# LoganWilliams1/mhm2_kmer_analysis_v2

Measured on AMD Instinct MI355X. Metric: k-mers/sec (kcount stage) at k=21, higher is better.
Workload: dtype u64

## Files before the change

### mhm2_kmer_analysis_v2_amd/csrc/kc_bucketed.hpp

```cpp
#pragma once
#include "kc_kernels.hpp"

namespace kc {

constexpr int WGB = 1024;
constexpr int SUPER_SPAN = 16 * WGB - PRE - POST;
using TileSuper = TileGeo<WGB, SUPER_SPAN>;
static_assert(TileSuper::GPT == 1 && TileSuper::NGROUP == WGB, "one group per thread");
constexpr int PMAX = 1024;
constexpr int GMAX = 512;

template <int NL> struct Rnd {
  static constexpr int RPOS = NL == 1 ? 16 : NL == 2 ? 8 : 4;
  static constexpr int RPOS_READS = NL == 1 ? 8 : NL <= 3 ? 4 : 2;
  static constexpr size_t STAGE = ((size_t)WGB * RPOS + 64) * NL * 8;
  static constexpr size_t STAGE_READS = ((size_t)WGB * RPOS_READS + 64) * NL * 8;
};

struct Geom {
  uint32_t G, P1, P2, S;
  uint32_t log2CH1, log2CH2;
  uint32_t L1MAX, L2MAX;
  uint32_t A1;
  uint32_t A2;
// ... 1327 lines not shown
  const uint32_t CH1m = (1u << gm.log2CH1) - 1u;
  const uint8_t *const rec1 = reinterpret_cast<const uint8_t *>(bb.rec1);
  for (uint32_t b1 = (FL ? fs.b_lo : 0u) + blockIdx.x; b1 < (FL ? fs.b_hi : P1); b1 += gridDim.x) {
    {
      const int tid = fresh_tid();
      uint32_t v = 0;
      if ((uint32_t)tid < G) {
        const uint32_t cnt = bb.cnt1[(size_t)tid * P1 + b1];
        uint32_t d = 0;
        if constexpr (INC) {
          d = bb.done1[(size_t)tid * P1 + b1];
          L.skip[tid] = d;
        }
        L.end[tid] = cnt;
        v = cnt > d ? ((cnt - (d & ~1u) + 1u) & ~1u) : 0u;
      }
      if constexpr (FL) {
        if ((uint32_t)tid >= G && (uint32_t)tid < GT) {
          const uint32_t c = fs.cnt[(size_t)(tid - G) * fs.nbo + (b1 - fs.b_lo)];
          L.flo[tid - G] = fs.at[(size_t)(tid - G) * fs.nbo + (b1 - fs.b_lo)];
          L.end[tid] = c;
          v = (c + 1u) & ~1u;
        }
      }
      const uint32_t e = block_excl_scan(v, L.sp.scan);
      if ((uint32_t)tid < GT) L.pre[tid] = e;
      if (tid == 0) L.pre[GT] = L.sp.scan.total;
    }
    ChainDest D;
    D.arena = bb.rec2;
    D.chain = bb.chain2 + (size_t)b1 * P2 * gm.L2MAX;
    D.log2CH = gm.log2CH2;
    D.LMAX = gm.L2MAX;
    D.arena_base = (uint32_t)__builtin_amdgcn_readfirstlane((int)bb.base2[b1]);
    D.arena_cap = (uint32_t)__builtin_amdgcn_readfirstlane((int)(bb.base2[b1 + 1] - bb.base2[b1]));
    D.own_lo = 0;
    D.own_hi = PMAX;
#ifdef KC_STAMPS
    unsigned long long tprev_ = __builtin_amdgcn_s_memtime();
    D.stamps = cb + 8;
    D.tprev = &tprev_;
#endif
    ChainState cst = split_load_state(L.sp, P2, INC ? bb.cnt2 + (size_t)b1 * P2 : nullptr, D.chain, D.LMAX, D.log2CH, INC ? bb.used2[b1] : 0u);
    __syncthreads();
    const uint32_t n = L.pre[GT];
    const uint32_t half = WGB * RPOS;
    uint32_t p_ids = 0, p_rec = 0;
    uint32_t nxa[NPAIR], nxb[NPAIR], nxc[NPAIR];
    uint32_t nxt_valid = 0, nxt_flat = 0;
    auto load_half = [&](uint32_t v0) __attribute__((always_inline)) {
      const uint32_t t = (uint32_t)fresh_tid();
      uint32_t ids[NPAIR];
#pragma unroll
      for (int j = 0; j < NPAIR; j++) {
        const uint32_t e = min(v0 + 2u * ((uint32_t)j * WGB + t), n - 2u);
        while (e >= L.pre[p_ids + 1]) p_ids++;
        const uint32_t i0 = e - L.pre[p_ids] + (INC ? (L.skip[p_ids] & ~1u) : 0u);
        const size_t ci = ((size_t)p_ids * gm.P1 + b1) * gm.L1MAX + (i0 >> gm.log2CH1);
        ids[j] = bb.chain1[FL && p_ids >= G ? 0 : ci];
      }
      nxt_valid = 0;
#pragma unroll
      for (int j = 0; j < NPAIR; j++) {
        const uint32_t ev = v0 + 2u * ((uint32_t)j * WGB + t), e = min(ev, n - 2u);
        while (e >= L.pre[p_rec + 1]) p_rec++;
        const bool flat = FL && p_rec >= G;
        const uint32_t first = (INC && !flat) ? L.skip[p_rec] : 0u;
        const uint32_t i0 = e - L.pre[p_rec] + (first & ~1u), end = L.end[p_rec];
        const uint8_t *src = rec1 + ((((size_t)p_rec * gm.A1 + ids[j]) << gm.log2CH1) + (i0 & CH1m)) * 6;
        if constexpr (FL) {
          const uint64_t f0 = L.flo[flat ? p_rec - G : 0u];
          if (flat) src = reinterpret_cast<const uint8_t *>((uintptr_t)f0) + 5u * (size_t)i0;
          nxt_flat = flat ? (nxt_flat | (1u << j)) : (nxt_flat & ~(1u << j));
        }
        const bool in = ev < n;
        nxt_valid |= (in && i0 >= first && i0 < end ? 1u : 0u) << (2 * j);
        nxt_valid |= (in && i0 + 1u < end ? 2u : 0u) << (2 * j);
        const Load12 w = *reinterpret_cast<const Load12 *>(src);
        nxa[j] = w.a;
        nxb[j] = w.b;
        nxc[j] = w.c;
      }
    };
    auto request = [&](uint64_t v0) __attribute__((always_inline)) {
      if (v0 < n) load_half((uint32_t)v0);
      else nxt_valid = 0;
    };
    uint32_t lo[RPOS], br[RPOS];
    uint32_t cur_valid = 0;
    const uint32_t sh_b2 = gm.k2 - gm.la - gm.lb;
    auto take_over = [&]() __attribute__((always_inline)) {
#pragma unroll
      for (int j = 0; j < NPAIR; j++) {
        const Load12 w = {nxa[j], nxb[j], nxc[j]};
        uint32_t e0, e1;
        if (FL && ((nxt_flat >> j) & 1u)) {
          lo[2 * j] = w.a;
          e0 = w.b & 63u;
          lo[2 * j + 1] = (w.b >> 8) | (w.c << 24);
          e1 = (w.c >> 8) & 63u;
        } else {
          lo[2 * j] = w.a;
          e0 = (w.b >> 10) & 63u;
          lo[2 * j + 1] = (w.b >> 16) | (w.c << 16);
          e1 = w.c >> 26;
        }
        br[2 * j] = ((lo[2 * j] >> sh_b2) & (P2 - 1u)) | (e0 << 10);
        br[2 * j + 1] = ((lo[2 * j + 1] >> sh_b2) & (P2 - 1u)) | (e1 << 10);
      }
      cur_valid = nxt_valid;
    };
    auto rank_half = [&](int buf) __attribute__((always_inline)) {
#pragma unroll
      for (int j = 0; j < RPOS; j++) {
        const bool valid = (cur_valid >> j) & 1u;
        const uint32_t rank = hist_rank(L.sp, buf, br[j] & (PMAX - 1), valid);
        br[j] = valid ? (br[j] | (rank << 16)) : ~0u;
      }
    };
    const uint32_t rb_mask = (1u << sh_b2) - 1u;
    auto scatter_half = [&](const uint32_t *at) __attribute__((always_inline)) {
#pragma unroll
      for (int j0 = 0; j0 < RPOS; j0 += 8) {
        uint32_t pos[8];
#pragma unroll
        for (int j = 0; j < 8; j++) pos[j] = at[br[j0 + j] & (PMAX - 1)];
#pragma unroll
        for (int j = 0; j < 8; j++) {
          const uint32_t bj = br[j0 + j];
          const uint32_t p = bj != ~0u ? pos[j] + (bj >> 16) : L2R6_ROUND + lane_id();
          staged[p] = ((lo[j0 + j] & rb_mask) << 6) | ((bj >> 10) & 63u);
        }
      }
    };
    uint32_t *const arena32 = reinterpret_cast<uint32_t *>(D.arena);
    const size_t arena0 = (size_t)D.arena_base << D.log2CH;
    if (n) load_half(0);
    take_over();
    request(half);
    int buf = 0;
    bool second = false;
    uint32_t a1 = 0, total1 = 0;
    for (uint32_t v0 = 0; v0 < n || second; v0 += half) {
      rank_half(buf);
      KC_SPLIT_STAMP(0)
      lds_barrier();
      uint32_t S = 0, o_hi = 0;
      {
        const int tid = fresh_tid();
        KC_SPLIT_STAMP(1)
        const uint32_t c = (uint32_t)tid < P2 ? L.sp.hist[buf][tid] : 0u;
        const uint32_t e = block_excl_scan(c, L.sp.scan);
        if (!second) {
          if ((uint32_t)tid < P2) L.sp.hist[buf ^ 1][tid] = e;
          a1 = c | (e << 16);
        } else {
          S = e;
          o_hi = (uint32_t)__builtin_amdgcn_readlane((int)(e + c), 63);
          if ((uint32_t)tid < P2) {
            const RunPlace q = split_reserve(L.sp, (uint32_t)tid, c, S, D, cst);
            L.sp.dst[tid] = make_uint4(q.x, q.y, q.fit | (q.w << 16), a1);
            L.sp.hist[buf][tid] = total1 + S - (a1 >> 16) - (a1 & 0xFFFFu);
            L.sp.hist[buf ^ 1][tid] = 0;
          }
        }
        lds_barrier();
        if (!second) total1 = (uint32_t)__builtin_amdgcn_readfirstlane((int)L.sp.scan.total);
        KC_SPLIT_STAMP(2)
      }
      scatter_half(second ? L.sp.hist[buf] : L.sp.hist[buf ^ 1]);
      if (second) lds_barrier();
      KC_SPLIT_STAMP(3)
      take_over();
      request(v0 + 2 * (uint64_t)half);
      KC_SPLIT_STAMP(5)
      if (second) {
        const int tid = fresh_tid();
        const uint32_t wave = (uint32_t)__builtin_amdgcn_readfirstlane(tid >> 6), lane = lane_id();
        uint32_t r0 = wave * 64u, Sl = S;
        if (P2 < (uint32_t)WGB) {
          if ((uint32_t)tid < P2) L.sp.hist[buf][tid] = S;
          lds_barrier();
          const uint32_t G = (P2 + 15u) >> 4, total = L.sp.scan.total;
          r0 = min(wave * G, P2);
          const uint32_t r1 = min(r0 + G, P2), r = min(r0 + lane, r1);
          Sl = r < r1 ? L.sp.hist[buf][r] : ~0u;
          o_hi = (uint32_t)__builtin_amdgcn_readfirstlane((int)(r1 < P2 ? L.sp.hist[buf][r1] : total));
        }
        const uint32_t o_lo = (uint32_t)__builtin_amdgcn_readlane((int)Sl, 0);
        constexpr int U = 4;
        for (uint32_t o0 = o_lo; o0 < o_hi; o0 += U * 64) {
          uint32_t oc[U], r[U], s[U], word[U];
          uint4 d[U];
#pragma unroll
          for (int u = 0; u < U; u++) {
            const uint32_t ou = min(o0 + 64u * u, o_hi - 1u);
            oc[u] = min(ou + lane, o_hi - 1u);
            const uint64_t le = __ballot(Sl <= ou);
            uint32_t l = 63u - (uint32_t)__clzll((long long)le);
            r[u] = l;
            s[u] = (uint32_t)__builtin_amdgcn_readlane((int)Sl, (int)l);
            for (uint64_t m = __ballot(Sl > ou && Sl - ou < 64u); m; m &= m - 1u) {
              l = (uint32_t)__builtin_ctzll(m);
              const uint32_t sl = (uint32_t)__builtin_amdgcn_readlane((int)Sl, (int)l);
              if (oc[u] >= sl) {
                r[u] = l;
                s[u] = sl;
              }
            }
          }
#pragma unroll
          for (int u = 0; u < U; u++) d[u] = L.sp.dst[r0 + r[u]];
#pragma unroll
          for (int u = 0; u < U; u++) {
            const uint32_t j = oc[u] - s[u], n1 = d[u].w & 0xFFFFu, st1 = d[u].w >> 16;
            word[u] = staged[j < n1 ? st1 + j : total1 + oc[u] - st1 - n1];
          }
          bool spill = false;
#pragma unroll
          for (int u = 0; u < U; u++) {
            const uint32_t j = oc[u] - s[u];
            const bool live = o0 + 64u * u + lane < o_hi, fits = j < (d[u].z & 0xFFFFu);
            const uint32_t at = (j < (d[u].z >> 16) ? d[u].x : d[u].y) + oc[u];
            if (live && fits) arena32[arena0 + at] = word[u];
            spill |= live && !fits;
          }
          if (__any(spill)) {
#pragma unroll
            for (int u = 0; u < U; u++) {
              if (o0 + 64u * u + lane < o_hi && oc[u] - s[u] >= (d[u].z & 0xFFFFu)) {
                const size_t reg = (size_t)b1 * P2 + r0 + r[u];
                bb.flag[reg] = 1;
                const uint64_t o = atomicAdd((unsigned long long *)&cb[CB_OVF2], 1ULL);
                if (o < bb.ovf2_cap) bb.ovf2[o] = cp_unpack_rec(word[u], reg, gm);
                else atomicOr((unsigned long long *)&cb[CB_FATAL], (unsigned long long)FATAL_OVF2);
              }
            }
          }
        }
        KC_SPLIT_STAMP(4)
        buf ^= 1;
      }
      second = !second;
    }
    {
      const int tid = fresh_tid();
      if ((uint32_t)tid < P2) bb.cnt2[(size_t)b1 * P2 + tid] = cst.cur;
      if constexpr (INC) {
        if ((uint32_t)tid < G) bb.done1[(size_t)tid * P1 + b1] = L.end[tid];
        if (tid == 0) bb.used2[b1] = min(L.sp.arena_used, D.arena_cap);
      }
    }
    __syncthreads();
  }
}

template <int NL, bool CP>
__global__ void kc_ovf1_to_regions_kernel(Geom gm, BucketBufs bb, uint64_t n, uint64_t *cb) {
  const uint64_t i = (uint64_t)blockIdx.x * blockDim.x + threadIdx.x;
  if (i >= n) return;
  uint64_t r[NL];
  for (int w = 0; w < NL; w++) r[w] = bb.ovf1[i * NL + w];
  size_t reg;
  if (CP) {
    const uint64_t m = cp_mix_rec(r[0], gm);
    reg = (size_t)cp_b1(m, gm) * gm.P2 + cp_b2(m, gm);
  } else {
    const uint64_t h = rec_hash<NL>(r);
    reg = (size_t)hash_b1(h, gm) * gm.P2 + hash_b2(h, gm);
  }
  bb.flag[reg] = 1;
  const uint64_t o = atomicAdd((unsigned long long *)&cb[CB_OVF2], 1ULL);
  if (o < bb.ovf2_cap) {
    for (int w = 0; w < NL; w++) bb.ovf2[o * NL + w] = r[w];
  } else {
    atomicOr((unsigned long long *)&cb[CB_FATAL], (unsigned long long)FATAL_OVF2);
  }
}

template <int NL, bool CP>
__global__ __launch_bounds__(TPB) void kc_ovf1_drain_kernel(Geom gm, BucketBufs bb, uint64_t n, Table t, uint64_t *ctrs) {
  for (uint64_t i = (uint64_t)blockIdx.x * TPB + threadIdx.x; i < n; i += (uint64_t)gridDim.x * TPB) {
    uint64_t r[NL];
    for (int w = 0; w < NL; w++) r[w] = bb.ovf1[i * NL + w];
    size_t reg;
    if (CP) {
      const uint64_t m = cp_mix_rec(r[0], gm);
      reg = (size_t)cp_b1(m, gm) * gm.P2 + cp_b2(m, gm);
    } else {
      const uint64_t h = rec_hash<NL>(r);
      reg = (size_t)hash_b1(h, gm) * gm.P2 + hash_b2(h, gm);
    }
    bb.flag[reg] = 1;
    table_insert<NL>(t, r, ctrs);
  }
}

constexpr uint32_t CHAIN_LDS = 480;

template <int NL>
struct CountLDS {
  static constexpr uint32_t SMAX = NL <= 2 ? 4096 : 2048;
  static constexpr int ew(bool) { return NL == 1 ? 6 : 5; }
  uint32_t chain[2][CHAIN_LDS];
  uint32_t hdr[2][2];
  uint32_t nout;
  uint32_t ncand;
  uint32_t fail[2];
  uint32_t gbase_lo, gbase_hi, gbase2_lo, gbase2_hi, split;
  static constexpr size_t header_bytes() { return (sizeof(CountLDS<NL>) + 15) & ~size_t(15); }
  static constexpr size_t bytes(uint32_t S, bool cp) { return header_bytes() + (size_t)S * ((cp ? 4 : 8 * NL) + 4 * ew(cp) + 2) + 16; }
};
static_assert(2 * CountLDS<2>::bytes(2048, false) <= 160 * 1024, "two workgroups of the two-word count kernel per CU");

struct CountTab {
  uint64_t *keys;
  uint32_t *ext;
  uint16_t *cand;
  uint32_t S, lgS;
};

template <int NL, bool CP>
__device__ __forceinline__ CountTab count_tab(uint8_t *smem, uint32_t S) {
  CountTab t;
  uint8_t *p = smem + CountLDS<NL>::header_bytes();
  t.keys = reinterpret_cast<uint64_t *>(p);
  p += (size_t)S * (CP ? 4 : 8 * NL);
  t.ext = reinterpret_cast<uint32_t *>(p);
  p += (size_t)S * 4 * CountLDS<NL>::ew(CP);
  t.cand = reinterpret_cast<uint16_t *>(p);
  t.S = S;
  t.lgS = 31u - (uint32_t)__clz(S);
  return t;
}

template <int EW>
__device__ __forceinline__ void ext_count(const CountTab &tb, uint32_t s, uint32_t le, uint32_t re) {
  if constexpr (EW == 6) {
    le = min(le, 4u);
    re = min(re, 4u);
    atomicAdd(&tb.ext[((le >> 1) << tb.lgS) + s], 1u << ((le & 1u) << 4));
    atomicAdd(&tb.ext[((3u + (re >> 1)) << tb.lgS) + s], 1u << ((re & 1u) << 4));
  } else {
    const bool nl = (le & 4u) != 0, nr = (re & 4u) != 0;
    const uint32_t wl = nl ? 4u : (le >> 1), wr = nr ? 4u : 2u + (re >> 1);
    const uint32_t il = nl ? 1u : 1u << ((le & 1u) << 4), ir = nr ? 0x10000u : 1u << ((re & 1u) << 4);
    atomicAdd(&tb.ext[(wl << tb.lgS) + s], il);
    atomicAdd(&tb.ext[(wr << tb.lgS) + s], ir);
  }
}
template <int EW>
__device__ __forceinline__ uint32_t ext_get(const uint32_t *ext, uint32_t SM, uint32_t s, uint32_t side, uint32_t e) {
  return (ext[((EW == 6 ? 3 : 2) * side + (e >> 1)) * SM + s] >> (16 * (e & 1u))) & 0xFFFFu;
}

struct OutBufs {
  uint64_t *keys;
  uint16_t *counts;
  uint8_t *left, *right;
  uint16_t *exts;
  uint64_t cap;
  uint64_t *cursor;
  uint32_t block;
  uint64_t *tails;
};

__device__ __forceinline__ uint32_t lds_probe1(unsigned long long *claim, uint32_t Sm1, uint64_t key, uint32_t slot, uint32_t valid,
                                               uint32_t &failed) {
  uint32_t act = valid;
  const uint32_t klo = (uint32_t)key, khi = (uint32_t)(key >> 32);
  uint32_t trips = 0;
  do {
    unsigned long long old = key;
    if (act) old = atomicCAS(&claim[slot], (unsigned long long)KEY_EMPTY, (unsigned long long)key);
    const uint32_t olo = (uint32_t)old, ohi = (uint32_t)(old >> 32);
    const uint32_t differs = (olo ^ klo) | (ohi ^ khi);
    const uint32_t notempty = ~(olo & ohi);
    const uint32_t miss = min(differs, notempty) ? act : 0u;
    act = miss;
    slot = (slot + miss) & Sm1;
    if (++trips > Sm1 + 1) {
      failed |= act;
      break;
    }
  } while (__any(act));
  return slot;
}

__device__ __forceinline__ uint32_t lds_probe32(uint32_t *claim, uint32_t Sm1, uint32_t key, uint32_t slot, uint32_t stride, bool valid,
                                                uint32_t &failed) {
#ifndef KC_PROBE_CXX
  uint32_t at = slot << 2, old, addr, trips = Sm1 + 2;
  const uint32_t m4 = Sm1 << 2, step = stride << 2;
  const uint32_t base = (uint32_t)(uintptr_t)claim;
  const uint64_t live = __builtin_amdgcn_ballot_w64(valid);
  uint64_t sv, t;
  asm volatile(
      "s_mov_b64 %[sv], exec\n\t"
      "s_and_b64 exec, exec, %[live]\n\t"
      "s_cbranch_execz 2f\n"
      "1:\n\t"
      "v_add_u32_e32 %[addr], %[base], %[at]\n\t"
      "ds_cmpst_rtn_b32 %[old], %[addr], %[empty], %[key]\n\t"
      "s_waitcnt lgkmcnt(0)\n\t"
      "v_cmp_ne_u32_e32 vcc, %[old], %[key]\n\t"
      "v_cmp_ne_u32_e64 %[t], -1, %[old]\n\t"
      "s_and_b64 vcc, vcc, %[t]\n\t"
      "s_and_b64 exec, exec, vcc\n\t"
      "s_cbranch_execz 2f\n\t"
      "v_add_u32_e32 %[at], %[step], %[at]\n\t"
      "v_and_b32_e32 %[at], %[m4], %[at]\n\t"
      "s_sub_u32 %[trips], %[trips], 1\n\t"
      "s_cmp_lg_u32 %[trips], 0\n\t"
      "s_cbranch_scc1 1b\n\t"
      "v_mov_b32_e32 %[fl], 1\n"
      "2:\n\t"
      "s_mov_b64 exec, %[sv]\n\t"
      : [old] "=&v"(old), [addr] "=&v"(addr), [at] "+v"(at), [fl] "+v"(failed), [trips] "+s"(trips), [sv] "=&s"(sv), [t] "=&s"(t)
      : [live] "s"(live), [base] "s"(base), [empty] "v"(0xFFFFFFFFu), [key] "v"(key), [step] "v"(step), [m4] "s"(m4)
      : "vcc", "scc", "memory");
  return at >> 2;
#else
  uint32_t trips = 0, at = slot << 2;
  const uint32_t m4 = Sm1 << 2, step = stride << 2;
  bool go = valid;
  do {
    uint32_t old = key;
    if (go) old = atomicCAS(reinterpret_cast<uint32_t *>(reinterpret_cast<char *>(claim) + at), 0xFFFFFFFFu, key);
    go = go & (old != key) & (old != 0xFFFFFFFFu);
    at = (at + (go ? step : 0u)) & m4;
    if (++trips > Sm1 + 1) {
      failed |= go ? 1u : 0u;
      break;
    }
  } while (__builtin_amdgcn_ballot_w64(go) != 0);
  return at >> 2;
#endif
}

template <int NL>
__device__ __forceinline__ uint32_t lds_probeN(const CountTab &tb, const uint64_t (&key)[NL], uint32_t slot, uint32_t valid, uint32_t &failed);

__device__ __forceinline__ uint32_t lds_probe2(const CountTab &tb, uint64_t key0, uint64_t klast, uint32_t slot, bool valid, uint32_t &failed) {
#ifndef KC_PROBE2_CXX
  const uint32_t m8 = (tb.S - 1u) << 3;
  uint32_t at = slot << 3, a0, a1, trips = 4u * tb.S + 2u;
  const uint32_t base0 = (uint32_t)(uintptr_t)tb.keys, base1 = base0 + (tb.S << 3);
  const uint64_t live = __builtin_amdgcn_ballot_w64(valid);
  const uint64_t empty = KEY_EMPTY, busy = KEY_BUSY;
  uint64_t old, w0, sv, act, won, t1, t2;
  asm volatile(
      "s_mov_b64 %[sv], exec\n\t"
      "s_and_b64 %[act], exec, %[live]\n\t"
      "s_mov_b64 exec, %[act]\n\t"
      "s_cbranch_execz 2f\n"
      "1:\n\t"
      "v_add_u32_e32 %[a1], %[base1], %[at]\n\t"
      "v_add_u32_e32 %[a0], %[base0], %[at]\n\t"
      "ds_cmpst_rtn_b64 %[old], %[a1], %[empty], %[busy]\n\t"
      "ds_read_b64 %[w0], %[a0]\n\t"
      "s_waitcnt lgkmcnt(0)\n\t"
      "v_cmp_eq_u64_e64 %[won], %[old], %[empty]\n\t"
      "s_and_b64 exec, %[act], %[won]\n\t"
      "ds_write_b64 %[a0], %[key0]\n\t"
      "ds_write_b64 %[a1], %[klast]\n\t"
      "s_mov_b64 exec, %[act]\n\t"
      "v_cmp_eq_u64_e64 %[t1], %[old], %[klast]\n\t"
      "v_cmp_eq_u64_e64 %[t2], %[w0], %[key0]\n\t"
      "s_and_b64 %[t1], %[t1], %[t2]\n\t"
      "s_or_b64 %[t1], %[t1], %[won]\n\t"
      "s_andn2_b64 %[act], %[act], %[t1]\n\t"
      "s_mov_b64 exec, %[act]\n\t"
      "s_cbranch_execz 2f\n\t"
      "v_cmp_ne_u64_e64 %[t2], %[old], %[busy]\n\t"
      "s_and_b64 exec, %[act], %[t2]\n\t"
      "v_add_u32_e32 %[at], 8, %[at]\n\t"
      "v_and_b32_e32 %[at], %[m8], %[at]\n\t"
      "s_mov_b64 exec, %[act]\n\t"
      "s_sub_u32 %[trips], %[trips], 1\n\t"
      "s_cmp_lg_u32 %[trips], 0\n\t"
      "s_cbranch_scc1 1b\n\t"
      "v_mov_b32_e32 %[fl], 1\n"
      "2:\n\t"
      "s_mov_b64 exec, %[sv]\n\t"
      : [old] "=&v"(old), [w0] "=&v"(w0), [a0] "=&v"(a0), [a1] "=&v"(a1), [at] "+v"(at), [fl] "+v"(failed), [trips] "+s"(trips), [sv] "=&s"(sv),
        [act] "=&s"(act), [won] "=&s"(won), [t1] "=&s"(t1), [t2] "=&s"(t2)
      : [live] "s"(live), [base0] "s"(base0), [base1] "s"(base1), [empty] "v"(empty), [busy] "v"(busy), [key0] "v"(key0), [klast] "v"(klast),
        [m8] "s"(m8)
      : "vcc", "scc", "memory");
  return at >> 3;
#else
  const uint64_t key[2] = {key0, klast};
  return lds_probeN<2>(tb, key, slot, valid ? 1u : 0u, failed);
#endif
}

template <int NL>
__device__ __forceinline__ uint32_t lds_probeN(const CountTab &tb, const uint64_t (&key)[NL], uint32_t slot, uint32_t valid, uint32_t &failed) {
  const uint32_t SM = tb.S, Sm1 = tb.S - 1u;
  unsigned long long *claim = (unsigned long long *)&tb.keys[(NL - 1) * SM];
  const unsigned long long klast = key[NL - 1];
  uint32_t act = valid, trips = 0;
  do {
    unsigned long long old;
    uint32_t won, same;
    if constexpr (NL >= 3) {
      old = atomicCAS(&claim[slot], act ? (unsigned long long)KEY_EMPTY : (unsigned long long)KEY_NEVER, (unsigned long long)KEY_BUSY);
      uint64_t other[NL > 1 ? NL - 1 : 1];
#pragma unroll
      for (int j = 0; j < NL - 1; j++) other[j] = tb.keys[j * SM + slot];
      won = (act && old == KEY_EMPTY) ? 1u : 0u;
      if (won) {
#pragma unroll
        for (int j = 0; j < NL - 1; j++) tb.keys[j * SM + slot] = key[j];
        __threadfence_block();
        atomicExch(&claim[slot], klast);
      }
      same = (old == klast || !act) ? 1u : 0u;
#pragma unroll
      for (int j = 0; j < NL - 1; j++) same &= (other[j] == key[j] || !act) ? 1u : 0u;
    } else {
      old = klast;
      if (act) old = atomicCAS(&claim[slot], (unsigned long long)KEY_EMPTY, (unsigned long long)KEY_BUSY);
      won = (act && old == KEY_EMPTY) ? 1u : 0u;
      if (won) {
#pragma unroll
        for (int j = 0; j < NL - 1; j++) tb.keys[j * SM + slot] = key[j];
        __threadfence_block();
        atomicExch(&claim[slot], klast);
      }
      same = old == klast ? 1u : 0u;
#pragma unroll
      for (int j = 0; j < NL - 1; j++) same &= (tb.keys[j * SM + slot] == key[j]) ? 1u : 0u;
    }
    const uint32_t busy = old == KEY_BUSY ? 1u : 0u;
    const uint32_t hit = won | same;
    const uint32_t miss = act & ~hit & ~busy & 1u;
    act &= ~hit & 1u;
    slot = (slot + miss) & Sm1;
    if (++trips > 4u * (Sm1 + 1u)) {
      failed |= act;
      break;
    }
  } while (__any(act));
  return slot;
}

constexpr uint32_t CHAIN_PRE = 64;
template <int NL, bool DUMP, bool CP>
__global__ __launch_bounds__(WGB, 8) void kc_count_kernel(Geom gm, BucketBufs bb, OutBufs out, int dmin_thres, uint64_t *ctrs,
                                                       uint64_t *cb) {
  extern __shared__ __align__(16) uint8_t smem[];
  CountLDS<NL> &T = *reinterpret_cast<CountLDS<NL> *>(smem);
  const int tid = threadIdx.x;
  const uint32_t S = gm.S, SM = gm.S;
  constexpr int EW = CountLDS<NL>::ew(CP);
  const CountTab tb = count_tab<NL, CP>(smem, S);
  const size_t R = (size_t)gm.P1 * gm.P2;
#ifdef KC_STAMPS
  unsigned long long tacc[6] = {0, 0, 0, 0, 0, 0}, tprev = __builtin_amdgcn_s_memtime();
  const bool stamp = tid == 0;
#define KC_STAMP(k)                                             \
  if (stamp) {                                                  \
    const unsigned long long tn = __builtin_amdgcn_s_memtime(); \
    tacc[k] += tn - tprev;                                      \
    tprev = tn;                                                 \
  }
#else
#define KC_STAMP(k)
#endif
  uint32_t *const keys32 = reinterpret_cast<uint32_t *>(tb.keys);
  auto reset_slot = [&](uint32_t s) {
    if (CP) {
      keys32[s] = 0xFFFFFFFFu;
    } else {
#pragma unroll
      for (int w = 0; w < NL; w++) tb.keys[w * SM + s] = KEY_EMPTY;
    }
#pragma unroll
    for (int e = 0; e < EW; e++) tb.ext[e * SM + s] = 0;
  };
  for (uint32_t s = tid; s < S; s += WGB) reset_slot(s);
  if (tid == 0) {
    T.nout = 0;
    T.ncand = 0;
    T.fail[0] = T.fail[1] = 0;
  }
  uint64_t cur_base = 0, cur_left = 0, sp_base = 0, sp_left = 0;
  bool pending = false;
  auto settle = [&]() {
    if (!pending) return;
    pending = false;
    uint64_t need = T.nout;
    T.nout = 0;
    if (need <= cur_left) {
      cur_base += need;
      cur_left -= need;
    } else {
      need -= cur_left;
      cur_base = sp_base + need;
      cur_left = sp_left - need;
      sp_base = sp_left = 0;
    }
  };
  uint32_t acc_entries = 0, acc_kept = 0;
  unsigned long long acc_sum = 0;
  uint32_t sink = 0;
  size_t r = blockIdx.x;
  int buf = 0;
  const uint32_t npre = min(CHAIN_PRE, gm.L2MAX);
  auto header_word = [&](size_t reg) -> uint32_t {
    const uint32_t *src = (uint32_t)tid < npre ? bb.chain2 + reg * gm.L2MAX + tid : (uint32_t)tid == npre ? bb.cnt2 + reg : bb.flag + reg;
    return *src;
  };
  auto header_park = [&](int b, uint32_t v) {
    if ((uint32_t)tid < npre) T.chain[b][tid] = v;
    else T.hdr[b][tid - npre] = v;
  };
  if (r < R && (uint32_t)tid < npre + 2u) header_park(0, header_word(r));
  __syncthreads();
  const uint32_t CHm = (1u << gm.log2CH2) - 1u;
  while (r < R) {
    const size_t rn = r + gridDim.x;
    const bool has_next = rn < R;
    uint32_t c_nxt = 0;
    if (has_next && (uint32_t)tid < npre + 2u) c_nxt = header_word(rn);
    const uint32_t n = T.hdr[buf][0], f_cur = T.hdr[buf][1];
    const bool process = n != 0 && f_cur == 0 && n <= KC_COUNT_MAX;
    if (n > KC_COUNT_MAX && f_cur == 0 && tid == 0) bb.flag[r] = 2;
    if (process) {
      if (tid == 0) {
        settle();
        T.ncand = 0;
        const uint64_t most = DUMP ? min(n, S) : min(n >> 1, S);
        if (out.block != 0) {
          if (cur_left + sp_left < most) {
            const uint64_t take = ((uint64_t)S + out.block - 1) / out.block * out.block;
            sp_base = atomicAdd((unsigned long long *)out.cursor, (unsigned long long)take);
            sp_left = take;
          }
          T.gbase_lo = (uint32_t)cur_base;
          T.gbase_hi = (uint32_t)(cur_base >> 32);
          T.gbase2_lo = (uint32_t)sp_base;
          T.gbase2_hi = (uint32_t)(sp_base >> 32);
          T.split = (uint32_t)min(cur_left, (uint64_t)0xFFFFFFFFu);
        }
        pending = true;
      }
      const uint32_t nch = (n + CHm) >> gm.log2CH2;
      if (nch > npre) {
        for (uint32_t i = npre + tid; i < nch; i += WGB) T.chain[buf][i] = bb.chain2[r * gm.L2MAX + i];
        __syncthreads();
      }
      KC_STAMP(0)
      constexpr int BATCH = NL == 2 ? 4 : 2;
      if constexpr (NL == 1 && CP) {
        uint32_t failed = 0;
        for (uint32_t i0 = 0; i0 < n; i0 += 2u * WGB) {
          uint32_t i = i0 + 2u * (uint32_t)tid;
          const bool v0 = i < n, v1 = i + 1u < n;
          i = v0 ? i : 0u;
          const size_t at = ((size_t)T.chain[buf][i >> gm.log2CH2] << gm.log2CH2) + (i & CHm);
          const uint2 rr = *reinterpret_cast<const uint2 *>(reinterpret_cast<const uint32_t *>(bb.rec2) + at);
          if (__builtin_amdgcn_ballot_w64(v0) == 0) continue;
#pragma unroll
          for (int j = 0; j < 2; j++) {
            const bool v = j ? v1 : v0;
            const uint32_t r0 = j ? rr.y : rr.x, key = r0 >> 6;
            const uint32_t s = lds_probe32(keys32, S - 1u, key, key & (S - 1u), ((key >> tb.lgS) << 1) | 1u, v, failed);
            const uint32_t le = r0 & 7u, re = (r0 >> 3) & 7u;
            if (v) ext_count<EW>(tb, s, le, re);
          }
        }
        if (failed) T.fail[buf] = 1;
      } else
      for (uint32_t i0 = 0; i0 < n; i0 += WGB * BATCH) {
        uint64_t rec[BATCH][NL];
        size_t at[BATCH];
#pragma unroll
        for (int j = 0; j < BATCH; j++) {
          uint32_t i = i0 + (uint32_t)j * WGB + tid;
          i = i < n ? i : 0u;
          at[j] = ((size_t)T.chain[buf][i >> gm.log2CH2] << gm.log2CH2) + (i & CHm);
        }
#pragma unroll
        for (int j = 0; j < BATCH; j++) {
#pragma unroll
          for (int w = 0; w < NL; w++) rec[j][w] = bb.rec2[at[j] * NL + w];
        }
        if constexpr (NL == 1) {
          uint32_t failed = 0;
#pragma unroll
          for (int j = 0; j < BATCH; j++) {
            const uint32_t v = (i0 + (uint32_t)j * WGB + tid) < n ? 1u : 0u;
            const uint64_t r0 = rec[j][0], key = r0 & ~KC_EXT_MASK;
            uint64_t kk[1] = {key};
            if (!__any(v)) continue;
            const uint32_t s = lds_probe1((unsigned long long *)tb.keys, S - 1u, key, hash_slot(kc_hash<1>(kk), S), v, failed);
            const uint32_t le = (uint32_t)r0 & 7u, re = ((uint32_t)r0 >> 3) & 7u;
            if (v) ext_count<EW>(tb, s, le, re);
          }
          if (failed) T.fail[buf] = 1;
        } else {
          uint32_t failed = 0;
#pragma unroll
          for (int j = 0; j < BATCH; j++) {
            const uint32_t v = (i0 + (uint32_t)j * WGB + tid) < n ? 1u : 0u;
            if (!__any(v)) continue;
            uint64_t key[NL];
#pragma unroll
            for (int w = 0; w < NL; w++) key[w] = rec[j][w];
            const uint32_t le = (uint32_t)(rec[j][NL - 1] & 7u), re = (uint32_t)((rec[j][NL - 1] >> 3) & 7u);
            key[NL - 1] &= ~KC_EXT_MASK;
            uint32_t s;
            if constexpr (NL == 2) s = lds_probe2(tb, key[0], key[1], hash_slot(kc_hash<NL>(key), S), v != 0u, failed);
            else s = lds_probeN<NL>(tb, key, hash_slot(kc_hash<NL>(key), S), v, failed);
            if (v && !(failed & 1u)) ext_count<EW>(tb, s, le, re);
          }
          if (failed) T.fail[buf] = 1;
        }
      }
    }
    if (has_next && (uint32_t)tid < npre + 2u) header_park(buf ^ 1, c_nxt);
    __syncthreads();
    KC_STAMP(1)
    if (process) {
      uint32_t touch = 0;
      if (has_next) {
        const uint32_t n_nxt = T.hdr[buf ^ 1][0], f_nxt = T.hdr[buf ^ 1][1];
        constexpr uint32_t PER_LINE = CP ? 32u : 16u / NL;
        const uint32_t i = (uint32_t)fresh_tid() * PER_LINE;
        if (f_nxt == 0 && n_nxt <= KC_COUNT_MAX && i < n_nxt && (i >> gm.log2CH2) < npre) {
          const size_t a = ((size_t)T.chain[buf ^ 1][i >> gm.log2CH2] << gm.log2CH2) + (i & CHm);
          touch = CP ? reinterpret_cast<const uint32_t *>(bb.rec2)[a] : (uint32_t)bb.rec2[a * NL];
        }
      }
      const bool failed = T.fail[buf] != 0;
      const uint64_t gbase = ((uint64_t)T.gbase_hi << 32) | T.gbase_lo, gbase2 = ((uint64_t)T.gbase2_hi << 32) | T.gbase2_lo;
      const uint32_t split = T.split;
      for (uint32_t s0 = 0; s0 < S; s0 += 2 * WGB) {
        uint32_t sx[2];
        bool in[2], taken[2], cand[2];
        uint32_t w[2][3];
#pragma unroll
        for (int u = 0; u < 2; u++) {
          sx[u] = s0 + (uint32_t)u * WGB + tid;
          in[u] = sx[u] < S;
          const uint32_t si = in[u] ? sx[u] : 0u;
          taken[u] = in[u] && (CP ? keys32[si] != 0xFFFFFFFFu : tb.keys[(NL - 1) * SM + si] != KEY_EMPTY);
          w[u][0] = tb.ext[si];
          w[u][1] = tb.ext[SM + si];
          w[u][2] = tb.ext[(EW == 5 ? 4 : 2) * SM + si];
        }
#pragma unroll
        for (int u = 0; u < 2; u++) {
          cand[u] = false;
          if (taken[u] && !failed) {
            const uint32_t count = (w[u][0] & 0xFFFFu) + (w[u][0] >> 16) + (w[u][1] & 0xFFFFu) + (w[u][1] >> 16) + (w[u][2] & 0xFFFFu);
            cand[u] = DUMP || count >= 2;
            acc_entries++;
          }
        }
        const uint64_t m0 = __ballot(cand[0]), m1 = __ballot(cand[1]);
        if (m0 | m1) {
          const uint32_t n0 = (uint32_t)__popcll(m0);
          uint32_t base = 0;
          if (lane_id() == 0) base = atomicAdd(&T.ncand, n0 + (uint32_t)__popcll(m1));
          base = __shfl(base, 0);
          const uint64_t below = (1ULL << lane_id()) - 1ULL;
          if (cand[0]) tb.cand[base + (uint32_t)__popcll(m0 & below)] = (uint16_t)sx[0];
          if (cand[1]) tb.cand[base + n0 + (uint32_t)__popcll(m1 & below)] = (uint16_t)sx[1];
        }
#pragma unroll
        for (int u = 0; u < 2; u++)
          if (taken[u] && !cand[u]) reset_slot(sx[u]);
      }
      __syncthreads();
      const uint32_t ncand = T.ncand;
      for (uint32_t i0 = 0; i0 < ncand; i0 += WGB) {
        const uint32_t i = i0 + tid;
        const bool live = i < ncand;
        const uint32_t s = live ? tb.cand[i] : 0u;
        bool keep = false;
        uint32_t count = 0, l = 0, rr = 0;
        uint32_t w[EW];
        if (live) {
#pragma unroll
          for (int x = 0; x < EW; x++) w[x] = tb.ext[x * SM + s];
          count = (w[0] & 0xFFFFu) + (w[0] >> 16) + (w[1] & 0xFFFFu) + (w[1] >> 16) + (w[EW == 5 ? 4 : 2] & 0xFFFFu);
          if (DUMP) {
            keep = true;
          } else {
            const uint32_t lc[4] = {w[0] & 0xFFFFu, w[0] >> 16, w[1] & 0xFFFFu, w[1] >> 16};
            constexpr int R0 = EW == 6 ? 3 : 2;
            const uint32_t rc[4] = {w[R0] & 0xFFFFu, w[R0] >> 16, w[R0 + 1] & 0xFFFFu, w[R0 + 1] >> 16};
            l = vote_ext(lc, count, dmin_thres);
            rr = vote_ext(rc, count, dmin_thres);
            keep = l < 4u && rr < 4u;
          }
        }
        const uint64_t m = __ballot(keep);
        if (m) {
          const int leader = __ffsll((long long)m) - 1;
          const uint32_t cnt = (uint32_t)__popcll(m);
          uint64_t o = 0;
          if (out.block != 0) {
            uint32_t base = 0;
            if ((int)lane_id() == leader) base = atomicAdd(&T.nout, cnt);
            base = __shfl(base, leader);
            const uint32_t rank = base + (uint32_t)__popcll(m & ((1ULL << lane_id()) - 1ULL));
            o = rank < split ? gbase + rank : gbase2 + (rank - split);
          } else {
            unsigned long long base = 0;
            if ((int)lane_id() == leader) base = atomicAdd((unsigned long long *)out.cursor, (unsigned long long)cnt);
            base = __shfl(base, leader);
            o = base + (uint64_t)__popcll(m & ((1ULL << lane_id()) - 1ULL));
          }
          if (keep && o < out.cap) {
            if (CP) {
              out.keys[o] = cp_unpack_rec(keys32[s] << 6, r, gm);
            } else {
#pragma unroll
              for (int x = 0; x < NL; x++) out.keys[o * NL + x] = tb.keys[x * SM + s];
            }
            out.counts[o] = (uint16_t)count;
            if (DUMP) {
              constexpr int R0 = EW == 6 ? 3 : 2;
#pragma unroll
              for (int x = 0; x < 4; x++) {
                out.exts[o * 8 + x] = (uint16_t)((w[x >> 1] >> (16 * (x & 1))) & 0xFFFFu);
                out.exts[o * 8 + 4 + x] = (uint16_t)((w[R0 + (x >> 1)] >> (16 * (x & 1))) & 0xFFFFu);
              }
            } else {
              out.left[o] = (uint8_t)("ACGT"[l & 3u]);
              out.right[o] = (uint8_t)("ACGT"[rr & 3u]);
            }
          }
          if (keep) {
            acc_kept++;
            acc_sum += count;
          }
        }
        if (live) reset_slot(s);
      }
      if (failed && tid == 0) {
        bb.flag[r] = 2;
        T.fail[buf] = 0;
      }
      sink ^= touch;
      __syncthreads();
      KC_STAMP(2)
    }
    r = rn;
    buf ^= 1;
  }
  if (tid == 0) {
    settle();
    if (out.block) {
      out.tails[4 * blockIdx.x] = cur_base;
      out.tails[4 * blockIdx.x + 1] = cur_left;
      out.tails[4 * blockIdx.x + 2] = sp_base;
      out.tails[4 * blockIdx.x + 3] = sp_left;
    }
  }
  if (!DUMP) {
    unsigned long long e = acc_entries, p = (unsigned long long)acc_entries - (unsigned long long)acc_kept, sm = acc_sum;
    for (int o = 32; o > 0; o >>= 1) {
      e += __shfl_down(e, o);
      p += __shfl_down(p, o);
      sm += __shfl_down(sm, o);
    }
    if (lane_id() == 0) {
      if (e) atomicAdd((unsigned long long *)&cb[CB_ENTRIES], e);
      if (p) atomicAdd((unsigned long long *)&ctrs[CTR_PURGED], p);
      if (sm) atomicAdd((unsigned long long *)&ctrs[CTR_SUM_COUNTS], sm);
    }
  }
  if (sink == 0x9E3779B9u && R == 0) cb[CB_DUMP] = sink;
#ifdef KC_STAMPS
  if (stamp)
    for (int k = 0; k < 5; k++) atomicAdd((unsigned long long *)&cb[8 + k], tacc[k]);
#endif
#undef KC_STAMP
}

constexpr uint32_t PLAN_RUNS = 1024;
constexpr size_t PLAN_WORDS = 4 + 4 * (size_t)(PLAN_RUNS + 1);

__global__ __launch_bounds__(WGB) void kc_out_plan_kernel(const uint64_t *tails, uint32_t nwg, uint64_t *cursor, uint64_t *reserved,
                                                        uint64_t *plan) {
  __shared__ uint64_t hs[PLAN_RUNS], hl[PLAN_RUNS];
  __shared__ uint32_t nh;
  const uint32_t tid = threadIdx.x;
  if (tid == 0) nh = 0;
  __syncthreads();
  uint64_t pos = 0, len = 0;
  if (tid < nwg) {
    pos = tails[2 * tid];
    len = tails[2 * tid + 1];
  }
  if (len) {
    uint32_t rank = 0;
    for (uint32_t j = 0; j < nwg; j++)
      if (tails[2 * j + 1] && tails[2 * j] < pos) rank++;
    hs[rank] = pos;
    hl[rank] = len;
    atomicAdd(&nh, 1u);
  }
  __syncthreads();
  if (tid == 0) {
    const uint64_t T = *cursor;
    uint64_t holes = 0;
    for (uint32_t i = 0; i < nh; i++) holes += hl[i];
    const uint64_t n = T - holes;
    uint64_t *hrun = plan + 4, *srun = plan + 4 + 2 * (PLAN_RUNS + 1);
    uint64_t nhole = 0, nsrc = 0, hcount = 0, scount = 0;
    uint64_t at = n;
    for (uint32_t i = 0; i < nh; i++) {
      const uint64_t b = hs[i], e = hs[i] + hl[i];
      if (b < n) {
        const uint64_t ee = e < n ? e : n;
        hrun[2 * nhole] = b;
        hrun[2 * nhole + 1] = hcount;
        hcount += ee - b;
        nhole++;
      }
      if (e > n) {
        const uint64_t bb = b > n ? b : n;
        if (bb > at) {
          srun[2 * nsrc] = at;
          srun[2 * nsrc + 1] = scount;
          scount += bb - at;
          nsrc++;
        }
        at = e;
      }
    }
    if (T > at) {
      srun[2 * nsrc] = at;
      srun[2 * nsrc + 1] = scount;
      scount += T - at;
      nsrc++;
    }
    hrun[2 * nhole + 1] = hcount;
    srun[2 * nsrc + 1] = scount;
    plan[0] = hcount < scount ? hcount : scount;
    plan[1] = nhole;
    plan[2] = nsrc;
    *reserved = T;
    *cursor = n;
  }
}

template <int NL>
__global__ void kc_out_move_kernel(const uint64_t *plan, OutBufs out) {
  const uint64_t nmove = plan[0];
  const uint32_t nhole = (uint32_t)plan[1], nsrc = (uint32_t)plan[2];
  const uint64_t *hrun = plan + 4, *srun = plan + 4 + 2 * (PLAN_RUNS + 1);
  auto locate = [](const uint64_t *run, uint32_t nrun, uint64_t m) -> uint64_t {
    uint32_t lo = 0, hi = nrun;
    while (hi - lo > 1) {
      const uint32_t mid = (lo + hi) >> 1;
      if (run[2 * mid + 1] <= m) lo = mid; else hi = mid;
    }
    return run[2 * lo] + (m - run[2 * lo + 1]);
  };
  for (uint64_t m = (uint64_t)blockIdx.x * blockDim.x + threadIdx.x; m < nmove; m += (uint64_t)gridDim.x * blockDim.x) {
    const uint64_t d = locate(hrun, nhole, m), sidx = locate(srun, nsrc, m);
    if (d >= out.cap || sidx >= out.cap) continue;
#pragma unroll
    for (int w = 0; w < NL; w++) out.keys[d * NL + w] = out.keys[sidx * NL + w];
    out.counts[d] = out.counts[sidx];
    out.left[d] = out.left[sidx];
    out.right[d] = out.right[sidx];
  }
}

template <int NL, bool CP>
__global__ __launch_bounds__(TPB) void kc_flagged_to_table_kernel(Geom gm, BucketBufs bb, Table t, uint64_t *ctrs) {
  const size_t R = (size_t)gm.P1 * gm.P2;
  for (size_t r = blockIdx.x; r < R; r += gridDim.x) {
    if (!bb.flag[r]) continue;
    const uint32_t n = bb.cnt2[r];
    for (uint32_t i = threadIdx.x; i < n; i += TPB) {
      uint64_t rec[NL];
      if (CP) {
        rec[0] = cp_unpack_rec(*l2_record32(gm, bb, r, i), r, gm);
      } else {
        const uint64_t *src = l2_record<NL>(gm, bb, r, i);
        for (int w = 0; w < NL; w++) rec[w] = src[w];
      }
      table_insert<NL>(t, rec, ctrs);
    }
  }
}

template <int NL, bool CP>
__global__ __launch_bounds__(TPB) void kc_l1_to_table_kernel(Geom gm, BucketBufs bb, Table t, uint64_t *ctrs) {
  const size_t nseg = (size_t)gm.G * gm.P1;
  for (size_t sgi = blockIdx.x; sgi < nseg; sgi += gridDim.x) {
    const uint32_t n = bb.cnt1[sgi];
    const uint32_t g = (uint32_t)(sgi / gm.P1), b = (uint32_t)(sgi % gm.P1);
    for (uint32_t i = threadIdx.x; i < n; i += TPB) {
      uint64_t rec[NL];
      if (NL == 1 && CP && gm.rec6) {
        rec[0] = l1_record6(gm, bb, g, b, i);
      } else {
        const uint64_t *src = l1_record<NL>(gm, bb, g, b, i);
        for (int w = 0; w < NL; w++) rec[w] = src[w];
      }
      if (CP) rec[0] = cp_unmix_rec(rec[0], gm);
      table_insert<NL>(t, rec, ctrs);
    }
  }
}

__global__ void kc_sum_flagged_kernel(Geom gm, BucketBufs bb, uint64_t *cb) {
  const size_t R = (size_t)gm.P1 * gm.P2;
  unsigned long long acc = 0;
  for (size_t r = (size_t)blockIdx.x * blockDim.x + threadIdx.x; r < R; r += (size_t)gridDim.x * blockDim.x)
    if (bb.flag[r]) acc += bb.cnt2[r];
  for (int o = 32; o > 0; o >>= 1) acc += __shfl_down(acc, o);
  if (lane_id() == 0 && acc) atomicAdd((unsigned long long *)&cb[CB_FLAGGED_RECS], acc);
}

}
```

Before: 100.1 billion.

## Store per-slot extension counters contiguously in LDS instead of planar arrays

Switches the LDS extension-count table from a structure-of-arrays layout (word e of slot s at e*S+s) to an array-of-structures layout, with each slot's words stored contiguously at s*STR. For the 5-word case the word order changes so the N-count word sits at index 2 and the right-side counts start at index 3. Loads and clears of a slot can then use vector LDS accesses where the stride allows. Because the stride is odd (5 or 6 words), neighbouring threads hitting nearby slots may now collide on LDS banks, and the strides used here rarely allow the wide vector paths.

```diff
diff --git a/mhm2_kmer_analysis_v2_amd/csrc/kc_bucketed.hpp b/mhm2_kmer_analysis_v2_amd/csrc/kc_bucketed.hpp
--- a/mhm2_kmer_analysis_v2_amd/csrc/kc_bucketed.hpp
+++ b/mhm2_kmer_analysis_v2_amd/csrc/kc_bucketed.hpp
@@ -1653,6 +1653,8 @@
 struct CountLDS {
   static constexpr uint32_t SMAX = NL <= 2 ? 4096 : 2048;
   static constexpr int ew(bool) { return NL == 1 ? 6 : 5; }
+  static constexpr int stride(bool cp) { return ew(cp); }
+  static constexpr int r0(bool) { return 3; }
   uint32_t chain[2][CHAIN_LDS];
   uint32_t hdr[2][2];
   uint32_t nout;
@@ -1660,7 +1662,7 @@
   uint32_t fail[2];
   uint32_t gbase_lo, gbase_hi, gbase2_lo, gbase2_hi, split;
   static constexpr size_t header_bytes() { return (sizeof(CountLDS<NL>) + 15) & ~size_t(15); }
-  static constexpr size_t bytes(uint32_t S, bool cp) { return header_bytes() + (size_t)S * ((cp ? 4 : 8 * NL) + 4 * ew(cp) + 2) + 16; }
+  static constexpr size_t bytes(uint32_t S, bool cp) { return header_bytes() + (size_t)S * ((cp ? 4 : 8 * NL) + 4 * stride(cp) + 2) + 16; }
 };
 static_assert(2 * CountLDS<2>::bytes(2048, false) <= 160 * 1024, "two workgroups of the two-word count kernel per CU");
 
@@ -1678,31 +1680,72 @@
   t.keys = reinterpret_cast<uint64_t *>(p);
   p += (size_t)S * (CP ? 4 : 8 * NL);
   t.ext = reinterpret_cast<uint32_t *>(p);
-  p += (size_t)S * 4 * CountLDS<NL>::ew(CP);
+  p += (size_t)S * 4 * CountLDS<NL>::stride(CP);
   t.cand = reinterpret_cast<uint16_t *>(p);
   t.S = S;
   t.lgS = 31u - (uint32_t)__clz(S);
   return t;
 }
 
-template <int EW>
+template <int EW, int STR, int R0>
 __device__ __forceinline__ void ext_count(const CountTab &tb, uint32_t s, uint32_t le, uint32_t re) {
+  uint32_t *const slot = tb.ext + __umul24(s, (uint32_t)STR);
   if constexpr (EW == 6) {
     le = min(le, 4u);
     re = min(re, 4u);
-    atomicAdd(&tb.ext[((le >> 1) << tb.lgS) + s], 1u << ((le & 1u) << 4));
-    atomicAdd(&tb.ext[((3u + (re >> 1)) << tb.lgS) + s], 1u << ((re & 1u) << 4));
+    atomicAdd(&slot[le >> 1], 1u << ((le & 1u) << 4));
+    atomicAdd(&slot[R0 + (re >> 1)], 1u << ((re & 1u) << 4));
   } else {
     const bool nl = (le & 4u) != 0, nr = (re & 4u) != 0;
-    const uint32_t wl = nl ? 4u : (le >> 1), wr = nr ? 4u : 2u + (re >> 1);
+    const uint32_t wl = nl ? 2u : (le >> 1), wr = nr ? 2u : R0 + (re >> 1);
     const uint32_t il = nl ? 1u : 1u << ((le & 1u) << 4), ir = nr ? 0x10000u : 1u << ((re & 1u) << 4);
-    atomicAdd(&tb.ext[(wl << tb.lgS) + s], il);
-    atomicAdd(&tb.ext[(wr << tb.lgS) + s], ir);
-  }
-}
-template <int EW>
-__device__ __forceinline__ uint32_t ext_get(const uint32_t *ext, uint32_t SM, uint32_t s, uint32_t side, uint32_t e) {
-  return (ext[((EW == 6 ? 3 : 2) * side + (e >> 1)) * SM + s] >> (16 * (e & 1u))) & 0xFFFFu;
+    atomicAdd(&slot[wl], il);
+    atomicAdd(&slot[wr], ir);
+  }
+}
+template <int STR>
+__device__ __forceinline__ void ext_load_left(const uint32_t *slot, uint32_t (&w)[3]) {
+  if constexpr (STR % 4 == 0) {
+    const uint4 a = *reinterpret_cast<const uint4 *>(slot);
+    w[0] = a.x, w[1] = a.y, w[2] = a.z;
+  } else if constexpr (STR % 2 == 0) {
+    const uint2 a = *reinterpret_cast<const uint2 *>(slot);
+    w[0] = a.x, w[1] = a.y, w[2] = slot[2];
+  } else {
+    w[0] = slot[0], w[1] = slot[1], w[2] = slot[2];
+  }
+}
+template <int STR>
+__device__ __forceinline__ void ext_load(const uint32_t *slot, uint32_t (&w)[STR]) {
+  if constexpr (STR % 4 == 0) {
+#pragma unroll
+    for (int x = 0; x < STR; x += 4) {
+      const uint4 a = *reinterpret_cast<const uint4 *>(slot + x);
+      w[x] = a.x, w[x + 1] = a.y, w[x + 2] = a.z, w[x + 3] = a.w;
+    }
+  } else if constexpr (STR % 2 == 0) {
+#pragma unroll
+    for (int x = 0; x < STR; x += 2) {
+      const uint2 a = *reinterpret_cast<const uint2 *>(slot + x);
+      w[x] = a.x, w[x + 1] = a.y;
+    }
+  } else {
+#pragma unroll
+    for (int x = 0; x < STR; x++) w[x] = slot[x];
+  }
+}
+template <int STR>
+__device__ __forceinline__ void ext_clear(uint32_t *slot) {
+  if constexpr (STR % 4 == 0) {
+#pragma unroll
+    for (int x = 0; x < STR; x += 4) *reinterpret_cast<uint4 *>(slot + x) = make_uint4(0, 0, 0, 0);
+  } else if constexpr (STR % 2 == 0) {
+#pragma unroll
+    for (int x = 0; x < STR; x += 2) *reinterpret_cast<uint2 *>(slot + x) = make_uint2(0, 0);
+  } else {
+#pragma unroll
+    for (int x = 0; x < STR; x++) slot[x] = 0;
+  }
 }
 
 struct OutBufs {
@@ -1905,7 +1948,7 @@
   CountLDS<NL> &T = *reinterpret_cast<CountLDS<NL> *>(smem);
   const int tid = threadIdx.x;
   const uint32_t S = gm.S, SM = gm.S;
-  constexpr int EW = CountLDS<NL>::ew(CP);
+  constexpr int EW = CountLDS<NL>::ew(CP), STR = CountLDS<NL>::stride(CP), R0 = CountLDS<NL>::r0(CP);
   const CountTab tb = count_tab<NL, CP>(smem, S);
   const size_t R = (size_t)gm.P1 * gm.P2;
 #ifdef KC_STAMPS
@@ -1928,8 +1971,7 @@
 #pragma unroll
       for (int w = 0; w < NL; w++) tb.keys[w * SM + s] = KEY_EMPTY;
     }
-#pragma unroll
-    for (int e = 0; e < EW; e++) tb.ext[e * SM + s] = 0;
+    ext_clear<STR>(tb.ext + s * (uint32_t)STR);
   };
   for (uint32_t s = tid; s < S; s += WGB) reset_slot(s);
   if (tid == 0) {
@@ -2020,7 +2062,7 @@
             const uint32_t r0 = j ? rr.y : rr.x, key = r0 >> 6;
             const uint32_t s = lds_probe32(keys32, S - 1u, key, key & (S - 1u), ((key >> tb.lgS) << 1) | 1u, v, failed);
             const uint32_t le = r0 & 7u, re = (r0 >> 3) & 7u;
-            if (v) ext_count<EW>(tb, s, le, re);
+            if (v) ext_count<EW, STR, R0>(tb, s, le, re);
           }
         }
         if (failed) T.fail[buf] = 1;
@@ -2049,7 +2091,7 @@
             if (!__any(v)) continue;
             const uint32_t s = lds_probe1((unsigned long long *)tb.keys, S - 1u, key, hash_slot(kc_hash<1>(kk), S), v, failed);
             const uint32_t le = (uint32_t)r0 & 7u, re = ((uint32_t)r0 >> 3) & 7u;
-            if (v) ext_count<EW>(tb, s, le, re);
+            if (v) ext_count<EW, STR, R0>(tb, s, le, re);
           }
           if (failed) T.fail[buf] = 1;
         } else {
@@ -2066,7 +2108,7 @@
             uint32_t s;
             if constexpr (NL == 2) s = lds_probe2(tb, key[0], key[1], hash_slot(kc_hash<NL>(key), S), v != 0u, failed);
             else s = lds_probeN<NL>(tb, key, hash_slot(kc_hash<NL>(key), S), v, failed);
-            if (v && !(failed & 1u)) ext_count<EW>(tb, s, le, re);
+            if (v && !(failed & 1u)) ext_count<EW, STR, R0>(tb, s, le, re);
           }
           if (failed) T.fail[buf] = 1;
         }
@@ -2099,9 +2141,7 @@
           in[u] = sx[u] < S;
           const uint32_t si = in[u] ? sx[u] : 0u;
           taken[u] = in[u] && (CP ? keys32[si] != 0xFFFFFFFFu : tb.keys[(NL - 1) * SM + si] != KEY_EMPTY);
-          w[u][0] = tb.ext[si];
-          w[u][1] = tb.ext[SM + si];
-          w[u][2] = tb.ext[(EW == 5 ? 4 : 2) * SM + si];
+          ext_load_left<STR>(tb.ext + si * (uint32_t)STR, w[u]);
         }
 #pragma unroll
         for (int u = 0; u < 2; u++) {
@@ -2134,16 +2174,14 @@
         const uint32_t s = live ? tb.cand[i] : 0u;
         bool keep = false;
         uint32_t count = 0, l = 0, rr = 0;
-        uint32_t w[EW];
+        uint32_t w[STR];
         if (live) {
-#pragma unroll
-          for (int x = 0; x < EW; x++) w[x] = tb.ext[x * SM + s];
-          count = (w[0] & 0xFFFFu) + (w[0] >> 16) + (w[1] & 0xFFFFu) + (w[1] >> 16) + (w[EW == 5 ? 4 : 2] & 0xFFFFu);
+          ext_load<STR>(tb.ext + s * (uint32_t)STR, w);
+          count = (w[0] & 0xFFFFu) + (w[0] >> 16) + (w[1] & 0xFFFFu) + (w[1] >> 16) + (w[2] & 0xFFFFu);
           if (DUMP) {
             keep = true;
           } else {
             const uint32_t lc[4] = {w[0] & 0xFFFFu, w[0] >> 16, w[1] & 0xFFFFu, w[1] >> 16};
-            constexpr int R0 = EW == 6 ? 3 : 2;
             const uint32_t rc[4] = {w[R0] & 0xFFFFu, w[R0] >> 16, w[R0 + 1] & 0xFFFFu, w[R0 + 1] >> 16};
             l = vote_ext(lc, count, dmin_thres);
             rr = vote_ext(rc, count, dmin_thres);
@@ -2176,7 +2214,6 @@
             }
             out.counts[o] = (uint16_t)count;
             if (DUMP) {
-              constexpr int R0 = EW == 6 ? 3 : 2;
 #pragma unroll
               for (int x = 0; x < 4; x++) {
                 out.exts[o * 8 + x] = (uint16_t)((w[x >> 1] >> (16 * (x & 1))) & 0xFFFFu);
```

Result: no change. 99.86 billion (-0.2%).
